# alxfox/AR_Voxel_Project

Hardware: AMD Instinct MI355X
Metric: Mvoxel-views/s (voxels x views / s) + carve wall-time, 512^3 grid x 36 views (higher is better)
Workload: dtype u8; 1 GPU; synthetic sphere silhouettes, 512x512x512 grid, 36 views 640x480, per step: derive bit planes + summed-area tables from the resident u8 masks, then dense carve of a fresh model by all views; one step after the other; views=36, jobs_in_flight=1, parallelism=single GPU, collective=none, cull=True

## Files before the change

ar_voxel_project_amd/capi.py:

```python
from __future__ import annotations

import ctypes as C
import os
from typing import Optional, Sequence, Tuple

import numpy as np

_HERE = os.path.dirname(os.path.abspath(__file__))
LIB_PATH = os.environ.get("ARVX_LIB_PATH") or os.path.join(_HERE, "lib", "libarvx.so")

OCC = 1
SEEN = 2
CARVE_NO_CULL = 1
CARVE_STATS = 2
CARVE_FUSED = 8
CARVE_STREAM = 16
CARVE_FILTER = 64
CARVE_NO_STREAM = 32
CARVE_DENSE_CLASSIFY = 128
CARVE_WHOLE_ITEMS = 256
PATH_DENSE_CLASSIFY = 1
PATH_ITEM_SHARING = 2
PATH_FRESH = 4
PATH_LAZY_CODES = 8
# ... 15 lines not shown
SYMBOLS = [
    "arvx_version", "arvx_last_error", "arvx_device_count", "arvx_projection_assoc",
    "arvx_ctx_create_slab_halo",
    "arvx_set_projection_assoc", "arvx_ctx_set_projection_assoc", "arvx_ctx_projection_assoc",
    "arvx_selftest_project", "arvx_selftest_depth", "arvx_selftest_view_tables",
    "arvx_ctx_create", "arvx_ctx_create_slab", "arvx_ctx_create_striped", "arvx_ctx_destroy",
    "arvx_ctx_set_stream", "arvx_ctx_set_exchange_stream", "arvx_ctx_synchronize", "arvx_ctx_voxels",
    "arvx_compose_projection", "arvx_set_views", "arvx_set_views_device",
    "arvx_set_images", "arvx_state_reset", "arvx_state_upload",
    "arvx_state_download", "arvx_state_device_ptr", "arvx_state_upload_halo",
    "arvx_state_upload_planes", "arvx_state_download_planes", "arvx_state_packet_geometry",
    "arvx_state_download_packets", "arvx_host_register",
    "arvx_host_unregister", "arvx_handle_unseen", "arvx_undistort", "arvx_undistort_device",
    "arvx_pack_occupancy", "arvx_pack_occupancy_global", "arvx_carve", "arvx_carve_views", "arvx_fast_carve",
    "arvx_color", "arvx_surface_count", "arvx_surface_download",
    "arvx_surface_depth_download", "arvx_color_samples",
    "arvx_color_visible", "arvx_surface_visible_download", "arvx_view_depth_download",
    "arvx_photo_carve", "arvx_carve_votes", "arvx_votes_download",
    "arvx_components", "arvx_components_download", "arvx_components_labels_download",
    "arvx_components_keep",
    "arvx_colors_upload", "arvx_closure", "arvx_closure_count", "arvx_closure_download",
    "arvx_closure_download32",
    "arvx_mc_cells", "arvx_mc_cells_download", "arvx_mc_mesh", "arvx_mc_mesh_download",
    "arvx_mc_mesh_download_faces", "arvx_mc_mesh_welded", "arvx_mc_mesh_welded_download",
    "arvx_mc_mesh_smooth", "arvx_mc_mesh_smooth_download",
    "arvx_mc_mesh_decimate", "arvx_mc_mesh_decimate_download",
    "arvx_render", "arvx_render_view", "arvx_render_download", "arvx_render_agreement",
    "arvx_occupancy_packet_words", "arvx_occupancy_compress", "arvx_occupancy_expand",
    "arvx_occupancy_expand_striped", "arvx_occupancy_pack_compress", "arvx_occupancy_expand_striped_others",
    "arvx_export_model", "arvx_get_stats", "arvx_last_carve_path", "arvx_last_fast_carve_path",
    "arvx_selftest_divide",
    "arvx_selftest_round",
    "arvx_ctx_set_rect_cache_limit", "arvx_selftest_rect_cache",
]


class ArvxError(RuntimeError):
    def __init__(self, code: int, msg: str):
        super().__init__(f"arvx error {code}: {msg}")
        self.code = code


class Stats(C.Structure):
    _fields_ = [
        ("subtiles", C.c_uint64),
        ("subtiles_carved", C.c_uint64),
        ("subtile_views_mixed", C.c_uint64),
        ("subtile_views_total", C.c_uint64),
        ("surface_voxels", C.c_uint64),
        ("reserved", C.c_uint64 * 3),
        ("host_total_fallbacks", C.c_uint64),
    ]


_libs: dict = {}
ASSOC_RIGHT, ASSOC_LEFT = 0, 1


def load_library(path: Optional[str] = None) -> C.CDLL:
    path = path or LIB_PATH
    if path in _libs:
        return _libs[path]
    if not os.path.exists(path):
        raise FileNotFoundError(
            f"{path} is missing: run `python -c 'import __graft_entry__ as g; g.build()'` "
            "(or make -C ar_voxel_project_amd/csrc); there is no CPU fallback")
# ... 38 lines not shown
        lib.arvx_state_download_packets.argtypes = [p, C.c_void_p, C.c_int64, C.c_void_p, C.c_int64,
                                                    C.POINTER(C.c_int64), C.POINTER(C.c_int64)]
        lib.arvx_host_register.argtypes = [C.c_void_p, C.c_size_t]
        lib.arvx_host_unregister.argtypes = [C.c_void_p]
        lib.arvx_handle_unseen.argtypes = [p]
    lib.arvx_state_upload_halo.argtypes = [p, u8p, u8p]
    lib.arvx_pack_occupancy.argtypes = [p, p]
    lib.arvx_pack_occupancy_global.argtypes = [p, p]
    lib.arvx_carve.argtypes = [p, C.c_uint]
    lib.arvx_carve_views.argtypes = [p, C.c_int, C.c_int, C.c_uint]
    lib.arvx_fast_carve.argtypes = [p]
    lib.arvx_color.argtypes = [p, C.c_int]
    lib.arvx_surface_count.argtypes = [p, C.POINTER(C.c_int64)]
    lib.arvx_surface_download.argtypes = [p, C.POINTER(C.c_int64), f32p]
    lib.arvx_surface_depth_download.argtypes = [p, f32p]
    lib.arvx_colors_upload.argtypes = [p, C.c_int64, C.POINTER(C.c_int64), f32p]
    lib.arvx_closure.argtypes = [p, C.c_int, C.c_int]
    lib.arvx_closure_count.argtypes = [p, C.POINTER(C.c_int64)]
    lib.arvx_closure_download.argtypes = [p, C.POINTER(C.c_int64), f32p]
    lib.arvx_export_model.argtypes = [p, f32p, C.c_int]
    lib.arvx_get_stats.argtypes = [p, C.POINTER(Stats)]
    if hasattr(lib, "arvx_last_carve_path"):
        lib.arvx_last_carve_path.argtypes = [p, C.POINTER(C.c_uint32)]
    if hasattr(lib, "arvx_last_fast_carve_path"):
        lib.arvx_last_fast_carve_path.argtypes = [p, C.POINTER(C.c_uint32)]
    ab_build = bool(os.environ.get("ARVX_LIB_PATH"))
    if hasattr(lib, "arvx_selftest_divide") or not ab_build:
        lib.arvx_selftest_divide.argtypes = [p, C.c_int64, f32p, f32p, f32p, f32p]
    if hasattr(lib, "arvx_selftest_round") or not ab_build:
        lib.arvx_selftest_round.argtypes = [p, C.POINTER(C.c_int64)]
    if hasattr(lib, "arvx_selftest_rect_cache") or not ab_build:
        lib.arvx_ctx_set_rect_cache_limit.argtypes = [p, C.c_uint64]
        lib.arvx_selftest_rect_cache.argtypes = [p, C.POINTER(C.c_int64)]
    if hasattr(lib, "arvx_mc_cells") or not ab_build:
        lib.arvx_mc_cells.argtypes = [p, C.POINTER(C.c_int64)]
        lib.arvx_mc_cells_download.argtypes = [p, C.POINTER(C.c_int32)]
    if hasattr(lib, "arvx_occupancy_compress") or not ab_build:
        lib.arvx_occupancy_packet_words.argtypes = [C.c_int64, C.c_int64]
        lib.arvx_occupancy_compress.argtypes = [p, C.c_void_p, C.c_int64, C.c_void_p, C.c_int64]
        lib.arvx_occupancy_expand.argtypes = [p, C.c_void_p, C.c_int, C.c_int, C.c_int64,
                                              C.c_int64, C.c_void_p, C.c_void_p]
        if hasattr(lib, "arvx_occupancy_expand_striped") or not ab_build:
            lib.arvx_occupancy_expand_striped.argtypes = [p, C.c_void_p, C.c_int, C.c_int64,
                                                          C.c_int64, C.c_int64, C.c_void_p,
                                                          C.c_void_p]
        if hasattr(lib, "arvx_occupancy_pack_compress"):
            lib.arvx_occupancy_pack_compress.argtypes = [p, C.c_void_p, C.c_int64, C.c_void_p]
            lib.arvx_occupancy_expand_striped_others.argtypes = [p, C.c_void_p, C.c_int, C.c_int, C.c_int64,
                                                                 C.c_int64, C.c_int64, C.c_void_p, C.c_void_p]
    if hasattr(lib, "arvx_mc_mesh_smooth"):
        lib.arvx_mc_mesh_smooth.argtypes = [p, C.c_int, C.c_float, C.c_float]
        lib.arvx_mc_mesh_smooth_download.argtypes = [p, C.c_void_p, C.c_void_p]
    if hasattr(lib, "arvx_mc_mesh_decimate"):
        lib.arvx_mc_mesh_decimate.argtypes = [p, C.c_int, C.c_int, C.POINTER(C.c_int64), C.POINTER(C.c_int64)]
        lib.arvx_mc_mesh_decimate_download.argtypes = [p, C.c_void_p, C.c_void_p, C.c_void_p, C.c_void_p,
                                                       C.c_void_p]
    if hasattr(lib, "arvx_color_visible"):
        lib.arvx_color_visible.argtypes = [p, C.c_int, C.c_float]
        lib.arvx_surface_visible_download.argtypes = [p, C.POINTER(C.c_int32)]
        lib.arvx_view_depth_download.argtypes = [p, C.c_int, f32p]
    if hasattr(lib, "arvx_photo_carve"):
        lib.arvx_photo_carve.argtypes = [p, C.c_float, C.c_int, C.c_float, C.c_int, C.POINTER(C.c_int),
                                         C.POINTER(C.c_int64)]
    if hasattr(lib, "arvx_carve_votes"):
        lib.arvx_carve_votes.argtypes = [p, C.c_int, C.c_uint]
        lib.arvx_votes_download.argtypes = [p, C.c_void_p, C.c_void_p]
# ... 16 lines not shown
            fn.restype = C.c_int64
        elif name not in ("arvx_last_error",):
            fn.restype = C.c_int
    _libs[path] = lib
    return lib


def occupancy_packet_words(n_words64: int, cap_words64: int) -> int:
    return int(load_library().arvx_occupancy_packet_words(n_words64, cap_words64))


def _check(rc: int, lib: Optional[C.CDLL] = None) -> None:
    if rc != 0:
        lib = lib or load_library()
        raise ArvxError(rc, lib.arvx_last_error().decode("utf-8", "replace"))


def _f32(a) -> np.ndarray:
    return np.ascontiguousarray(a, dtype=np.float32)


def _fp(a: np.ndarray):
    return a.ctypes.data_as(C.POINTER(C.c_float))


def compose_projection(K, Rt) -> np.ndarray:
    K = _f32(K).reshape(9)
    Rt = _f32(Rt).reshape(12)
    M = np.empty(12, np.float32)
    _check(load_library().arvx_compose_projection(_fp(K), _fp(Rt), _fp(M)))
    return M.reshape(3, 4)


def stripe_planes(Z: int, world: int, rank: int) -> np.ndarray:
    groups = np.arange(rank, Z // 8, world)
    return (groups[:, None] * 8 + np.arange(8)[None, :]).reshape(-1)


class Context:

    def __init__(self, X: int, Y: int, Z: int, voxel_size: float, device: int = 0,
                 z_range: Optional[Sequence[int]] = None,
                 stripes: Optional[Sequence[int]] = None, lib_path: Optional[str] = None,
                 assoc: Optional[int] = None, halo: int = 1):
        self._lib = load_library(lib_path)
        self._h = C.c_void_p()
        self.X, self.Y, self.Z = int(X), int(Y), int(Z)
        self.voxel_size = float(np.float32(voxel_size))
        if stripes is not None:
            world, rank = int(stripes[0]), int(stripes[1])
            self._ck(self._lib.arvx_ctx_create_striped(C.byref(self._h), device, X, Y, Z,
                                                     C.c_float(voxel_size), world, rank))
            self.planes = stripe_planes(Z, world, rank)
            self.z_range = None
        else:
            z0, z1 = (0, Z) if z_range is None else (int(z_range[0]), int(z_range[1]))
            self.z_range = (z0, z1)
            self._lib.arvx_ctx_create_slab_halo.argtypes = [
                C.POINTER(C.c_void_p), C.c_int, C.c_int, C.c_int, C.c_int, C.c_float, C.c_int,
                C.c_int, C.c_int]
            self._ck(self._lib.arvx_ctx_create_slab_halo(C.byref(self._h), device, X, Y, Z,
                                                       C.c_float(voxel_size), z0, z1, int(halo)))
            self.planes = np.arange(z0, z1)
        nz = len(self.planes)
        self.shape = (nz, Y, X)
        self.nvox = nz * Y * X
# ... 502 lines not shown
        return b, d, i

    def render_agreement(self, view: int) -> Tuple[int, int, int]:
        counts = (C.c_int64 * 3)()
        self._ck(self._lib.arvx_render_agreement(self._h, int(view), counts))
        self._render_wh = (self.W, self.H)
        return int(counts[0]), int(counts[1]), int(counts[2])

    def mc_mesh_count(self, apply_unseen: bool = False) -> int:
        n = C.c_int64()
        self._lib.arvx_mc_mesh.argtypes = [C.c_void_p, C.c_int, C.POINTER(C.c_int64)]
        self._ck(self._lib.arvx_mc_mesh(self._h, int(apply_unseen), C.byref(n)))
        return int(n.value)

    def export_model(self, apply_unseen: bool = False) -> np.ndarray:
        out = np.empty((self.nvox, 4), np.float32)
        self._ck(self._lib.arvx_export_model(self._h, _fp(out), int(apply_unseen)))
        return out

    def selftest_divide(self, a0, a1, b) -> np.ndarray:
        a0, a1, b = _f32(a0).reshape(-1), _f32(a1).reshape(-1), _f32(b).reshape(-1)
        out = np.empty((len(b), 4), np.float32)
        self._ck(self._lib.arvx_selftest_divide(self._h, len(b), _fp(a0), _fp(a1), _fp(b), _fp(out)))
        return out

    def selftest_round(self) -> int:
        n = C.c_int64(-1)
        self._ck(self._lib.arvx_selftest_round(self._h, C.byref(n)))
        return int(n.value)

    def set_rect_cache_limit(self, nbytes: int) -> None:
        self._ck(self._lib.arvx_ctx_set_rect_cache_limit(self._h, nbytes))

    def selftest_rect_cache(self) -> int:
        n = C.c_int64(-2)
        self._ck(self._lib.arvx_selftest_rect_cache(self._h, C.byref(n)))
        return int(n.value)

    def stats(self) -> dict:
        s = Stats()
        self._ck(self._lib.arvx_get_stats(self._h, C.byref(s)))
        out = {k: int(getattr(s, k)) for k, _ in Stats._fields_ if k != "reserved"}
        out["slices_evaluated"] = int(s.reserved[0])
        out["open_voxels_in_slices"] = int(s.reserved[1])
        out["mixed_pairs_uniform"] = int(s.reserved[2])
        out["host_total_fallbacks"] = int(s.host_total_fallbacks)
        return out
```

ar_voxel_project_amd/csrc/arvx_capi.hip:

```cpp
#include "arvx/arvx.h"

#include <hip/hip_runtime.h>

#include <cmath>
#include <cstdarg>
#include <cstdio>
#include <cstdlib>
#include <atomic>
#include <cstring>
#include <mutex>
#include <new>
#include <string>
#include <type_traits>
#include <utility>
#include <vector>

#include "arvx_ctx.h"
#include "carve_kernels.h"
#include "rect_cache_kernels.h"
#ifdef ARVX_EXPERIMENTS
#include "carve_stream_kernels.h"
#endif
#include "views_kernels.h"
#include "state_kernels.h"
// ... 486 lines not shown
    ARVX_SYNC(ctx);
    ctx->stream = hip_stream ? (hipStream_t)hip_stream : ctx->own_stream;
    ctx->carve_layout = 0;
    return ARVX_OK;
}

int arvx_ctx_set_exchange_stream(arvx_ctx *ctx, void *hip_stream) {
    ARVX_CHECK_CTX(ctx);
    ctx->xstream = (hipStream_t)hip_stream;
    return ARVX_OK;
}

#ifdef ARVX_EXPERIMENTS
extern "C" int arvx_experiment_mark_fault(arvx_ctx *ctx, unsigned mark) {
    if (!ctx || !ctx->h_fault) return fail(ARVX_ERR_INVALID, "null context");
    *ctx->h_fault = mark;
    return ARVX_OK;
}
#endif

int arvx_ctx_synchronize(arvx_ctx *ctx) {
    ARVX_CHECK_CTX(ctx);
    ARVX_HIP(hipStreamSynchronize(ctx->stream));
    return check_fault(ctx);
}

int arvx_ctx_voxels(const arvx_ctx *ctx, int64_t *count) {
    if (!ctx || !count) return fail(ARVX_ERR_INVALID, "null argument");
    *count = (int64_t)ctx->nvox;
    return ARVX_OK;
}


static int views_common(Ctx *ctx, int V, const float *M, const float *campos, int W, int H,
                        int C) {
    if (V < 1 || V > 4096) return fail(ARVX_ERR_INVALID, "V=%d out of range [1,4096]", V);
    if (!M) return fail(ARVX_ERR_INVALID, "null M");
    if (W < 1 || H < 1 || W > arvx::kMaxImageDim || H > arvx::kMaxImageDim)
        return fail(ARVX_ERR_INVALID, "image size %dx%d out of range", W, H);
    if (C < 1 || C > 4) return fail(ARVX_ERR_INVALID, "channels=%d out of range [1,4]", C);
    const bool same = ctx->M() && ctx->V == V && ctx->W == W && ctx->H == H;
    ctx->drop(Event::SetViews);
    ctx->views_ready = false;
    ctx->cameras_ready = false;
    if (!same) {
        ctx->free_views();
        ctx->pool_images.release();
    }
    ctx->images_ready = false;
    ctx->V = V;
    ctx->W = W;
    ctx->H = H;
    ctx->bgWords = (int)(((((size_t)W * H + 31) / 32 + 1) + 31) / 32 * 32);
    ctx->satW = (W + 1 + 63) / 64 * 64;
    ctx->satH = H + 1;
    ctx->satStride = ctx->satW * ctx->satH;
    if (!same) {
        hipError_t e = ctx->pool_M.reserve((size_t)V * 12 * sizeof(float));
        if (e == hipSuccess) e = ctx->pool_campos.reserve((size_t)V * 3 * sizeof(float));
        if (e == hipSuccess) e = ctx->pool_bg.reserve((size_t)V * ctx->bgWords * sizeof(uint32_t));
        if (e == hipSuccess) e = ctx->pool_sat.reserve((size_t)V * ctx->satStride * sizeof(uint16_t));
        if (e != hipSuccess) {
            ctx->free_views();
            return arvx::fail_hip(e, "hipMalloc(views)", __FILE__, __LINE__);
        }
    }
    const bool same_M = same && ctx->h_M.size() == (size_t)V * 12 &&
                        memcmp(ctx->h_M.data(), M, (size_t)V * 12 * sizeof(float)) == 0;
    if (!same_M) {
        ctx->rect_invalidate();
        ctx->h_M.assign(M, M + (size_t)V * 12);
        ARVX_HIP(hipMemcpyAsync(ctx->M(), ctx->h_M.data(), (size_t)V * 12 * sizeof(float),
                                hipMemcpyHostToDevice, ctx->stream));
    }
    ctx->has_campos = campos != nullptr;
    if (campos) {
        const bool same_c = same && ctx->h_campos.size() == (size_t)V * 3 &&
                            memcmp(ctx->h_campos.data(), campos, (size_t)V * 3 * sizeof(float)) == 0;
        if (!same_c) {
            ctx->h_campos.assign(campos, campos + (size_t)V * 3);
            ARVX_HIP(hipMemcpyAsync(ctx->campos(), ctx->h_campos.data(),
                                    (size_t)V * 3 * sizeof(float), hipMemcpyHostToDevice,
                                    ctx->stream));
        }
    } else {
        ctx->h_campos.clear();
    }
    return ARVX_OK;
}

static int views_preprocess(Ctx *ctx, const uint8_t *d_masks, int C) {
    const int npix = ctx->W * ctx->H;
    ARVX_HIP(hipGetLastError());
    static const bool three_launches = experiment_flag("ARVX_VIEWS_THREE_LAUNCHES");
    if ((C == 1 || C == 3) && ctx->W % 64 == 0 && ctx->W / 64 + 1 <= arvx::kStripMaxWaves && ctx->H <= 4096 &&
        ((uintptr_t)d_masks & 15u) == 0 && !three_launches) {
        const int TIs = (ctx->H + 63) / 64;
        const size_t G = (size_t)ctx->W / 2;
        const size_t off_gran = ((size_t)ctx->V * sizeof(unsigned long long) + 255) / 256 * 256;
        const size_t vbytes = off_gran + (size_t)ctx->V * TIs * G * sizeof(unsigned long long);
        const size_t key = ((size_t)ctx->V << 40) ^ ((size_t)TIs << 24) ^ G;
        if (ctx->vstrip_key != key || ctx->pool_vstrip.cap < vbytes) {
            ARVX_HIP(ctx->pool_vstrip.reserve(vbytes));
            ARVX_HIP(hipMemsetAsync(ctx->pool_vstrip.p, 0, vbytes, ctx->stream));
            ctx->vstrip_key = key;
        }
        unsigned long long *ctr = (unsigned long long *)ctx->pool_vstrip.p;
        unsigned long long *gran = (unsigned long long *)((uint8_t *)ctx->pool_vstrip.p + off_gran);
        if (C == 1)
            hipLaunchKernelGGL(arvx::views_strip_kernel<1>, dim3(TIs, ctx->V), dim3(64 * (ctx->W / 64 + 1)),
                               0, ctx->stream, d_masks, ctx->W, ctx->H, TIs, ctx->bg(), ctx->bgWords,
                               ctx->sat(), ctx->satStride, ctx->satW, ctr, gran, ctx->d_fault);
        else
            hipLaunchKernelGGL(arvx::views_strip_kernel<3>, dim3(TIs, ctx->V), dim3(64 * (ctx->W / 64 + 1)),
                               0, ctx->stream, d_masks, ctx->W, ctx->H, TIs, ctx->bg(), ctx->bgWords,
                               ctx->sat(), ctx->satStride, ctx->satW, ctr, gran, ctx->d_fault);
        ARVX_HIP(hipGetLastError());
        ctx->views_ready = true;
        ctx->cameras_ready = true;
        return ARVX_OK;
    }
    if (C == 1 && npix % 32 == 0 && ((uintptr_t)d_masks & 15u) == 0) {
        hipLaunchKernelGGL(arvx::views_bits16_kernel, dim3((npix / 16 + 255) / 256, ctx->V),
                           dim3(256), 0, ctx->stream, d_masks, npix, ctx->bg(), ctx->bgWords);
    } else if (C == 1 || C == 3) {
        const dim3 g1(((npix + 3) / 4 + 255) / 256, ctx->V);
        if (C == 1)
            hipLaunchKernelGGL(arvx::views_bits_kernel<1>, g1, dim3(256), 0, ctx->stream, d_masks,
                               npix, ctx->bg(), ctx->bgWords);
        else
            hipLaunchKernelGGL(arvx::views_bits_kernel<3>, g1, dim3(256), 0, ctx->stream, d_masks,
                               npix, ctx->bg(), ctx->bgWords);
    } else {
        const dim3 g1((npix + 255) / 256, ctx->V);
        hipLaunchKernelGGL(arvx::views_bits_generic_kernel, g1, dim3(256), 0, ctx->stream, d_masks,
                           C, npix, ctx->bg(), ctx->bgWords);
    }
    ARVX_HIP(hipGetLastError());
    const int W = ctx->W, H = ctx->H, V = ctx->V;
    const int TJ = (W + 1 + 63) / 64, TI = (H + arvx::kTileRows - 1) / arvx::kTileRows;
    const size_t n_rs = (size_t)V * H * TJ, n_T = (size_t)V * TI * TJ * 64, n_ts = (size_t)V * TI * TJ;
    ARVX_HIP(ctx->pool_scratch.reserve((n_rs + n_T + n_ts) * sizeof(int) + 64));
    int *d_rs = (int *)ctx->pool_scratch.p, *d_T = d_rs + n_rs, *d_ts = d_T + n_T;
    const unsigned tgrid = (unsigned)(((size_t)TJ * TI * V + 3) / 4);
    hipLaunchKernelGGL(arvx::views_tile_sums_kernel, dim3(tgrid), dim3(256), 0, ctx->stream,
                       ctx->bg(), ctx->bgWords, W, H, TJ, TI, V, d_rs, d_T, d_ts);
    hipLaunchKernelGGL(arvx::views_table_kernel, dim3(tgrid), dim3(256), 0, ctx->stream,
                       ctx->bg(), ctx->bgWords, W, H, TJ, TI, V, d_rs, d_T, d_ts, ctx->sat(),
                       ctx->satStride, ctx->satW);
    ARVX_HIP(hipGetLastError());
    ctx->views_ready = true;
    ctx->cameras_ready = true;
    return ARVX_OK;
}

int arvx_set_views(arvx_ctx *ctx, int V, const float *M, const float *campos,
                   const uint8_t *const *masks, int W, int H, int C, size_t stride) {
    ARVX_CHECK_CTX(ctx);
    if (!masks) {
        if (int rc0 = views_common(ctx, V, M, campos, W, H, C > 0 ? C : 1)) return rc0;
        ctx->cameras_ready = true;
        ARVX_SYNC(ctx);
        return ARVX_OK;
    }
    if (W >= 1 && C >= 1 && stride < (size_t)W * C)
        return fail(ARVX_ERR_INVALID, "stride %zu < W*C", stride);
    for (int i = 0; i < V; ++i)
        if (!masks[i]) return fail(ARVX_ERR_INVALID, "null mask %d", i);
    int rc = views_common(ctx, V, M, campos, W, H, C);
    if (rc) return rc;
    const size_t img = (size_t)W * H * C;
    ARVX_HIP(ctx->pool_raw_masks.reserve(img * V));
    uint8_t *d_raw = (uint8_t *)ctx->pool_raw_masks.p;
    bool packed = stride == (size_t)W * C;
    for (int i = 1; i < V && packed; ++i) packed = masks[i] == masks[i - 1] + img;
    if (packed) {
        ARVX_HIP(hipMemcpyAsync(d_raw, masks[0], img * V, hipMemcpyHostToDevice, ctx->stream));
    } else {
        for (int i = 0; i < V; ++i)
            ARVX_HIP(hipMemcpy2DAsync(d_raw + img * i, (size_t)W * C, masks[i], stride,
                                      (size_t)W * C, H, hipMemcpyHostToDevice, ctx->stream));
    }
    rc = views_preprocess(ctx, d_raw, C);
    if (rc) return rc;
    ARVX_SYNC(ctx);
// ... 1833 lines not shown
                          const int32_t *xyz, float *rows_uv) {
    ARVX_CHECK_CTX(ctx);
    if (!M) return fail(ARVX_ERR_INVALID, "null M");
    arvx::SelftestMatrix m;
    memcpy(m.m, M, sizeof m.m);
    const unsigned grid = (unsigned)((n + 255) / 256);
    return selftest_xyz(ctx, n, xyz, (size_t)n * 5, rows_uv, [&](int *d_xyz, float *d_out) {
        by_assoc(ctx, [&](auto left) {
            hipLaunchKernelGGL(arvx::selftest_project_kernel<decltype(left)::value>, dim3(grid), dim3(256), 0,
                               ctx->stream, m, voxel_size, d_xyz, (long long)n, d_out, d_out + 3 * n);
        });
    });
}

int arvx_selftest_depth(arvx_ctx *ctx, int64_t n, const float campos[3], float voxel_size,
                        const int32_t *xyz, float *depth) {
    ARVX_CHECK_CTX(ctx);
    if (!campos) return fail(ARVX_ERR_INVALID, "null campos");
    arvx::SelftestMatrix m;
    memset(&m, 0, sizeof m);
    memcpy(m.m, campos, 3 * sizeof(float));
    return selftest_xyz(ctx, n, xyz, (size_t)n, depth, [&](int *d_xyz, float *d_out) {
        hipLaunchKernelGGL(arvx::selftest_depth_kernel, dim3((unsigned)((n + 255) / 256)), dim3(256),
                           0, ctx->stream, m, voxel_size, d_xyz, (long long)n, d_out);
    });
}

int arvx_selftest_view_tables(arvx_ctx *ctx, int view, uint32_t *bg_bits, uint16_t *table, int *ld) {
    ARVX_CHECK_CTX(ctx);
    if (!ctx->views_ready) return fail(ARVX_ERR_STATE, "arvx_set_views has not been called");
    if (view < 0 || view >= ctx->V) return fail(ARVX_ERR_INVALID, "view %d outside [0,%d)", view, ctx->V);
    if (!ld) return fail(ARVX_ERR_INVALID, "null ld");
    *ld = ctx->satW;
    const size_t words = ((size_t)ctx->W * ctx->H + 31) / 32;
    if (bg_bits)
        ARVX_HIP(hipMemcpyAsync(bg_bits, ctx->bg() + (size_t)view * ctx->bgWords, words * sizeof(uint32_t),
                                hipMemcpyDeviceToHost, ctx->stream));
    if (table)
        ARVX_HIP(hipMemcpyAsync(table, ctx->sat() + (size_t)view * ctx->satStride,
                                (size_t)ctx->satStride * sizeof(uint16_t), hipMemcpyDeviceToHost,
                                ctx->stream));
    ARVX_SYNC(ctx);
    return ARVX_OK;
}

int arvx_selftest_round(arvx_ctx *ctx, int64_t *mismatches) {
    ARVX_CHECK_CTX(ctx);
    if (!mismatches) return fail(ARVX_ERR_INVALID, "null mismatches");
    *mismatches = -1;
    ARVX_HIP(ctx->pool_scratch.reserve(64));
    unsigned long long *d_bad = (unsigned long long *)ctx->pool_scratch.p;
    ARVX_HIP(hipMemsetAsync(d_bad, 0, sizeof *d_bad, ctx->stream));
    const unsigned ranges[2][2] = {{0x00000000u, 0x4B800000u}, {0x80000000u, 0xBEFFFFFFu}};
    for (const auto &r : ranges) {
        const unsigned long long n = (unsigned long long)r[1] - r[0] + 1;
        hipLaunchKernelGGL(arvx::selftest_round_kernel, dim3((unsigned)((n + 255) / 256)), dim3(256),
                           0, ctx->stream, r[0], r[1], d_bad);
        ARVX_HIP(hipGetLastError());
    }
    unsigned long long bad = 0;
    ARVX_HIP(hipMemcpyAsync(&bad, d_bad, sizeof bad, hipMemcpyDeviceToHost, ctx->stream));
    ARVX_SYNC(ctx);
    *mismatches = (int64_t)bad;
    return ARVX_OK;
}

int arvx_ctx_set_rect_cache_limit(arvx_ctx *ctx, uint64_t bytes) {
    ARVX_CHECK_CTX(ctx);
    if (bytes > (uint64_t)1 << 46) return fail(ARVX_ERR_INVALID, "limit of %llu bytes", (unsigned long long)bytes);
    if (ctx->pool_rect.p) ARVX_SYNC(ctx);
    ctx->pool_rect.release();
    ctx->rect_state = Ctx::Rect::None;
    ctx->rect_limit = (size_t)bytes;
    return ARVX_OK;
// ... 1028 lines not shown
```

ar_voxel_project_amd/csrc/arvx_ctx.h:

```cpp
#pragma once

#include <hip/hip_runtime.h>
#include <stdint.h>

#include <vector>

namespace arvx {

int fail_hip(hipError_t e, const char *what, const char *file, int line);
int fail_msg(int code, const char *msg);

#define ARVX_HIP(call)                                                        \
    do {                                                                      \
        hipError_t arvx_e_ = (call);                                          \
        if (arvx_e_ != hipSuccess)                                            \
            return ::arvx::fail_hip(arvx_e_, #call, __FILE__, __LINE__);      \
    } while (0)

struct DevPool {
    enum Size { Headroom, Exact };
    void *p = nullptr;
    size_t cap = 0;
    const bool exact;
    explicit DevPool(Size size = Headroom) : exact(size == Exact) {}
// ... 97 lines not shown
    int64_t timeline_n = 0;
    int timeline_rec = 32;
    DevPool pool_flood_rec{DevPool::Exact};
    DevPool pool_flood_code;
    DevPool pool_coarse{DevPool::Exact};
    DevPool pool_stats{DevPool::Exact};
    unsigned long long *stats() const { return (unsigned long long *)pool_stats.p; }
    unsigned long long host_total_fallbacks = 0;
    DevPool pool_scratch{DevPool::Exact};
    DevPool pool_xscratch;
    DevPool pool_flood{DevPool::Exact};

    bool views_ready = false;
    bool cameras_ready = false;
    bool has_campos = false;
    int V = 0, W = 0, H = 0;
    int bgWords = 0, satStride = 0;
    int satW = 0, satH = 0;
    DevPool pool_M{DevPool::Exact}, pool_campos{DevPool::Exact}, pool_bg{DevPool::Exact},
        pool_sat{DevPool::Exact};
    float *M() const { return (float *)pool_M.p; }
    float *campos() const { return (float *)pool_campos.p; }
    uint32_t *bg() const { return (uint32_t *)pool_bg.p; }
    uint16_t *sat() const { return (uint16_t *)pool_sat.p; }
    std::vector<float> h_M, h_campos;
    enum class Rect { None, Built, Refused };
    Rect rect_state = Rect::None;
    int rect_streak = 0;
    size_t rect_limit = (size_t)1 << 30;
    DevPool pool_rect{DevPool::Exact};
    void rect_invalidate() {
        rect_state = Rect::None;
        rect_streak = 0;
    }

    DevPool pool_images{DevPool::Exact};
    uint8_t *images() const { return (uint8_t *)pool_images.p; }
    bool images_ready = false;
    int *d_surf_index = nullptr;
    float4 *d_surf_rgba = nullptr;
    float *d_surf_depth = nullptr;
    uint8_t *d_surf_has = nullptr;
    int64_t surf_count = 0;
    std::vector<int> h_surf_index;
    std::vector<uint8_t> h_surf_has;
    bool color_ready = false;
    DevPool pool_col_bits, pool_col_rank;
    bool color_visible = false;
    long long vis_large_need = 0;
    DevPool pool_vis_depth{DevPool::Exact}, pool_vis_large{DevPool::Exact}, pool_vis_views;
    DevPool pool_photo_rm, pool_photo_plane{DevPool::Exact};
    DevPool pool_votes{DevPool::Exact};
    bool votes_ready = false;

    DevPool pool_comp_label{DevPool::Exact}, pool_comp_planes{DevPool::Exact}, pool_comp_rank{DevPool::Exact},
        pool_comp_table, pool_comp_ctl;
    bool comp_ready = false;
    int comp_conn = 0;
    long long comp_count = 0, comp_cap = 0;

    int *d_clo_index = nullptr;
    void *d_clo_rgba = nullptr;
    int64_t clo_count = 0;
    bool closure_ready = false;
    int closure_unseen = 0;
    bool closure_fills = false;
    int closure_radius = 0;
// ... 104 lines not shown
```

ar_voxel_project_amd/csrc/views_kernels.h:

```cpp
#pragma once

#include "arvx_device.h"

namespace arvx {

template <int C>
__global__ __launch_bounds__(256) void views_bits_kernel(const uint8_t *__restrict__ masks,
                                                         int npix, uint32_t *__restrict__ bg,
                                                         int bgWords) {
    const int v = blockIdx.y;
    const int q = blockIdx.x * 256 + threadIdx.x;
    uint32_t *dst = bg + (size_t)v * bgWords;
    if (q == 0) dst[bgWords - 1] = 0;
    const uint8_t *src = masks + ((size_t)v * npix + 4 * (size_t)q) * C;
    uint32_t nib = 0;
    if (4 * q + 3 < npix && (((uintptr_t)src) & 3u) == 0) {
        uint32_t w[C];
#pragma unroll
        for (int c = 0; c < C; ++c) w[c] = reinterpret_cast<const uint32_t *>(src)[c];
        const uint8_t *b = reinterpret_cast<const uint8_t *>(w);
#pragma unroll
        for (int j = 0; j < 4; ++j) {
            bool isbg = true;
#pragma unroll
// ... 185 lines not shown
        const uint32_t t = (((d[k] & 0x7f7f7f7fu) + 0x7f7f7f7fu) | d[k]) & 0x80808080u;
        f |= bytes_to_nibble(t >> 7) << (4 * k);
    }
    return f;
}
__device__ __forceinline__ uint32_t nonzero_bytes(const uint32_t x) {
    return ((((x & 0x7f7f7f7fu) + 0x7f7f7f7fu) | x) >> 7) & 0x01010101u;
}

__device__ __forceinline__ uint32_t nonzero16x3(const uint4 a, const uint4 b, const uint4 c) {
    const uint32_t d[12] = {a.x, a.y, a.z, a.w, b.x, b.y, b.z, b.w, c.x, c.y, c.z, c.w};
    uint32_t m[2] = {0u, 0u};
#pragma unroll
    for (int k = 0; k < 12; ++k) {
        const uint32_t t = (((d[k] & 0x7f7f7f7fu) + 0x7f7f7f7fu) | d[k]) & 0x80808080u;
        m[k / 6] |= bytes_to_nibble(t >> 7) << (4 * (k % 6));
    }
    uint32_t f = 0;
#pragma unroll
    for (int h = 0; h < 2; ++h) {
        uint32_t x = (m[h] | (m[h] >> 1) | (m[h] >> 2)) & 0x249249u;
        x = (x | (x >> 2)) & 0x0C30C3u;
        x = (x | (x >> 4)) & 0x00F00Fu;
        x = (x | (x >> 8)) & 0xFFu;
        f |= x << (8 * h);
    }
    return f;
}

template <int C>
__global__ __launch_bounds__(64 * kStripMaxWaves) void views_strip_kernel(
    const uint8_t *__restrict__ masks, int W, int H, int TI, uint32_t *__restrict__ bg, int bgWords,
    uint16_t *__restrict__ sat, int satStride, int ld, unsigned long long *__restrict__ ctr,
    unsigned long long *__restrict__ gran, unsigned *__restrict__ err) {
    __shared__ unsigned long long s_bits[64 * (kStripMaxWaves - 1)];
    __shared__ int s_rowcnt[kStripMaxWaves][64];
    __shared__ uint16_t s_col[kStripMaxWaves][64];
    __shared__ int s_tot[kStripMaxWaves];
    __shared__ uint4 s_row[kStripMaxWaves][64];
    __shared__ unsigned long long s_ticket;
    const int v = blockIdx.y;
    if (threadIdx.x == 0) s_ticket = atomicAdd(&ctr[v], 1ull);
    __syncthreads();
    const unsigned long long ticket = s_ticket;
    const int I = (int)(ticket % (unsigned long long)TI);
    const uint32_t tag = (uint32_t)(ticket / (unsigned long long)TI) + 1u;
    const int J = threadIdx.x >> 6, lane = threadIdx.x & 63;
    const int TP = W >> 6;
    const int G = W >> 1;
    const uint8_t *img = masks + (size_t)v * W * H * C;
    const int y0 = I * 64;
    const int nrows = min(64, H - y0);
    const int rr = lane >> 2, q = lane & 3;

    uint32_t mine_lo = 0, mine_hi = 0;
    uint32_t acc[4] = {0u, 0u, 0u, 0u};
    if (J < TP) {
        uint4 w[4][C];
#pragma unroll
        for (int k = 0; k < 4; ++k) {
            const int y = y0 + 4 * rr + k;
            const uint4 *src = reinterpret_cast<const uint4 *>(img + ((size_t)y * W + 64 * J + 16 * q) * C);
#pragma unroll
            for (int c = 0; c < C; ++c) w[k][c] = (y < H) ? src[c] : make_uint4(0u, 0u, 0u, 0u);
        }
#pragma unroll
        for (int k = 0; k < 4; ++k) {
// ... 64 lines not shown
    }

    int above = 0;
    if (J < TP && I > 0) {
        const unsigned long long *g0 = gran + (size_t)v * TI * G + 32 * J + (lane >> 1);
        for (unsigned spin = 0;; ++spin) {
            bool ok = true;
            int sum = 0;
            for (int k = 0; k < I; ++k) {
                const unsigned long long g = granule_load(g0 + (size_t)k * G);
                ok = ok && (uint32_t)(g >> 32) == tag;
                sum += (int)(((uint32_t)g >> (16 * (lane & 1))) & 0xffffu);
            }
            if (__all(ok)) {
                above = sum;
                break;
            }
            if (spin > (1u << 20)) {
                if (lane == 0) __hip_atomic_store(err, 1u, __ATOMIC_RELAXED, __HIP_MEMORY_SCOPE_SYSTEM);
                break;
            }
            __builtin_amdgcn_s_sleep(8);
        }
    }
    int sc = above;
#pragma unroll
    for (int d = 1; d < 64; d <<= 1) {
        const int t = __shfl_up(sc, d);
        if (lane >= d) sc += t;
    }
    if (lane == 63) s_tot[J] = sc;
    __syncthreads();

    int left = 0, lt = 0;
    for (int k = 0; k < J; ++k) {
        left += s_rowcnt[k][lane];
        lt += s_tot[k];
    }
    uint16_t *tab = sat + (size_t)v * satStride;
    const unsigned off = 64u * (unsigned)J + (unsigned)lane;
    if (I == 0) tab[off] = 0;
    uint4 *const rows = s_row[J];
    rows[lane] = make_uint4(mine_lo, mine_hi, (uint32_t)left, 0u);
    wave_lds_fence();
    uint32_t run = (uint32_t)(sc - above + lt);
    uint16_t *row = tab + (size_t)(y0 + 1) * ld;
#pragma unroll 4
    for (int r = 0; r < nrows; ++r) {
        const uint4 f = rows[r];
        run = __builtin_amdgcn_mbcnt_hi(f.y, __builtin_amdgcn_mbcnt_lo(f.x, run)) + f.z;
        row[off] = (uint16_t)run;
        row += ld;
    }
}

}
```

include/arvx/arvx.h:

```cpp
#ifndef ARVX_H
#define ARVX_H

#include <stddef.h>
#include <stdint.h>

#ifdef __cplusplus
extern "C" {
#endif

#define ARVX_VERSION 100

enum {
    ARVX_OK = 0,
    ARVX_ERR_INVALID = 1,
    ARVX_ERR_HIP = 2,
    ARVX_ERR_STATE = 3,
    ARVX_ERR_NOMEM = 4
};

#define ARVX_OCC 1u
#define ARVX_SEEN 2u

#define ARVX_CARVE_NO_CULL 1u
#define ARVX_CARVE_STATS 2u
// ... 160 lines not shown

int arvx_get_stats(arvx_ctx *ctx, arvx_stats *out);

#define ARVX_PATH_DENSE_CLASSIFY 1u
#define ARVX_PATH_ITEM_SHARING 2u
#define ARVX_PATH_FRESH 4u
#define ARVX_PATH_LAZY_CODES 8u
#define ARVX_PATH_FUSED 16u
#define ARVX_PATH_BRUTE_FORCE 32u
#define ARVX_PATH_STREAM 64u
#define ARVX_PATH_RECT_BLOCKS 128u
int arvx_last_carve_path(arvx_ctx *ctx, uint32_t out[4]);

#define ARVX_FLOOD_PREPASS 1u
#define ARVX_FLOOD_FRESH 2u
int arvx_last_fast_carve_path(arvx_ctx *ctx, uint32_t out[4]);

int arvx_selftest_divide(arvx_ctx *ctx, int64_t n, const float *a0, const float *a1,
                         const float *b, float *out);

int arvx_selftest_project(arvx_ctx *ctx, int64_t n, const float M[12], float voxel_size,
                          const int32_t *xyz, float *rows_uv);
int arvx_selftest_depth(arvx_ctx *ctx, int64_t n, const float campos[3], float voxel_size,
                        const int32_t *xyz, float *depth);

int arvx_selftest_view_tables(arvx_ctx *ctx, int view, uint32_t *bg_bits, uint16_t *table, int *ld);

int arvx_selftest_round(arvx_ctx *ctx, int64_t *mismatches);

int arvx_ctx_set_rect_cache_limit(arvx_ctx *ctx, uint64_t bytes);

int arvx_selftest_rect_cache(arvx_ctx *ctx, int64_t *mismatches);

#ifdef __cplusplus
}
#endif
#endif
```

Baseline: 52.77 million Mvoxel-views/s.

## Skip summed-area table writes outside each view's projected grid window

Computes a conservative per-view image window from the projection of the grid bounding box, with error margins, on the host. The window is cached and uploaded as packed tile ranges. The strip kernel then returns early for tiles outside that window, skipping their summed-area table row writes. Tables are marked partial and fully rebuilt from the bit planes when a caller downloads them. This trades host-side bound computation and extra bookkeeping for fewer table stores, and it relies on the carve never reading table entries outside the window.

```diff
diff --git a/ar_voxel_project_amd/capi.py b/ar_voxel_project_amd/capi.py
--- a/ar_voxel_project_amd/capi.py
+++ b/ar_voxel_project_amd/capi.py
@@ -71,6 +71,8 @@
     "arvx_selftest_divide",
     "arvx_selftest_round",
     "arvx_ctx_set_rect_cache_limit", "arvx_selftest_rect_cache",
+    "arvx_ctx_set_view_window", "arvx_view_window", "arvx_view_window_host",
+    "arvx_selftest_fill_view_tables", "arvx_selftest_view_table_raw",
 ]
 
 
@@ -175,6 +177,13 @@
     if hasattr(lib, "arvx_selftest_rect_cache") or not ab_build:
         lib.arvx_ctx_set_rect_cache_limit.argtypes = [p, C.c_uint64]
         lib.arvx_selftest_rect_cache.argtypes = [p, C.POINTER(C.c_int64)]
+    if hasattr(lib, "arvx_view_window") or not ab_build:
+        lib.arvx_ctx_set_view_window.argtypes = [p, C.c_int]
+        lib.arvx_view_window.argtypes = [p, C.c_int, C.POINTER(C.c_int)]
+        lib.arvx_view_window_host.argtypes = [C.c_int, C.c_int, C.c_int, C.c_float, f32p, C.c_int, C.c_int,
+                                              C.POINTER(C.c_int)]
+        lib.arvx_selftest_fill_view_tables.argtypes = [p, C.c_int]
+        lib.arvx_selftest_view_table_raw.argtypes = [p, C.c_int, C.c_void_p]
     if hasattr(lib, "arvx_mc_cells") or not ab_build:
         lib.arvx_mc_cells.argtypes = [p, C.POINTER(C.c_int64)]
         lib.arvx_mc_cells_download.argtypes = [p, C.POINTER(C.c_int32)]
@@ -257,6 +266,13 @@
     return M.reshape(3, 4)
 
 
+def view_window_host(X: int, Y: int, Z: int, voxel_size: float, M, W: int, H: int) -> Tuple[int, int, int, int]:
+    M = _f32(M).reshape(12)
+    rect = (C.c_int * 4)()
+    _check(load_library().arvx_view_window_host(X, Y, Z, C.c_float(voxel_size), _fp(M), W, H, rect))
+    return tuple(int(r) for r in rect)
+
+
 def stripe_planes(Z: int, world: int, rank: int) -> np.ndarray:
     groups = np.arange(rank, Z // 8, world)
     return (groups[:, None] * 8 + np.arange(8)[None, :]).reshape(-1)
@@ -825,6 +841,26 @@
     def set_rect_cache_limit(self, nbytes: int) -> None:
         self._ck(self._lib.arvx_ctx_set_rect_cache_limit(self._h, nbytes))
 
+    def set_view_window(self, on: bool) -> None:
+        self._ck(self._lib.arvx_ctx_set_view_window(self._h, int(bool(on))))
+
+    def view_window(self, view: int) -> Tuple[int, int, int, int]:
+        rect = (C.c_int * 4)()
+        self._ck(self._lib.arvx_view_window(self._h, view, rect))
+        return tuple(int(r) for r in rect)
+
+    def selftest_fill_view_tables(self, value: int) -> None:
+        self._ck(self._lib.arvx_selftest_fill_view_tables(self._h, int(value)))
+
+    def selftest_view_table_raw(self, view: int, H: int) -> np.ndarray:
+        ld = C.c_int()
+        self._lib.arvx_selftest_view_tables.argtypes = [C.c_void_p, C.c_int, C.c_void_p, C.c_void_p,
+                                                        C.POINTER(C.c_int)]
+        self._ck(self._lib.arvx_selftest_view_tables(self._h, view, None, None, C.byref(ld)))
+        table = np.zeros((H + 1, ld.value), np.uint16)
+        self._ck(self._lib.arvx_selftest_view_table_raw(self._h, view, table.ctypes.data))
+        return table
+
     def selftest_rect_cache(self) -> int:
         n = C.c_int64(-2)
         self._ck(self._lib.arvx_selftest_rect_cache(self._h, C.byref(n)))
diff --git a/ar_voxel_project_amd/csrc/arvx_capi.hip b/ar_voxel_project_amd/csrc/arvx_capi.hip
--- a/ar_voxel_project_amd/csrc/arvx_capi.hip
+++ b/ar_voxel_project_amd/csrc/arvx_capi.hip
@@ -542,6 +542,122 @@
 }
 
 
+static bool view_window(int X, int Y, int Z, float s, const float *M, int W, int H, int win[4]) {
+    const int TI = (H + 63) / 64, JL = W / 64;
+    win[0] = 0;
+    win[1] = TI - 1;
+    win[2] = 0;
+    win[3] = JL;
+    const double wy[2] = {0.0, (double)((float)(Y - 1) * s)};
+    const double wx[2] = {0.0, (double)((float)(X - 1) * s)};
+    const double wz[2] = {0.0, (double)((float)(-(Z - 1)) * s)};
+    double E[3], lo[3], hi[3];
+    double a[3][8];
+    for (int r = 0; r < 3; ++r) {
+        const double m0 = M[4 * r], m1 = M[4 * r + 1], m2 = M[4 * r + 2], m3 = M[4 * r + 3];
+        E[r] = std::fabs(m0) * std::fabs(wy[1]) + std::fabs(m1) * std::fabs(wx[1]) +
+               std::fabs(m2) * std::fabs(wz[1]) + std::fabs(m3);
+        for (int c = 0; c < 8; ++c) a[r][c] = m0 * wy[c & 1] + m1 * wx[(c >> 1) & 1] + m2 * wz[c >> 2] + m3;
+    }
+    double cmin = INFINITY, cmax = -INFINITY;
+    for (int c = 0; c < 8; ++c) {
+        cmin = std::fmin(cmin, a[2][c]);
+        cmax = std::fmax(cmax, a[2][c]);
+    }
+    const double k19 = 1.001 / 524288.0, k20 = 1.0 / 1048576.0, k12 = 1.0 / 4096.0;
+    const double eps0 = E[0] * k19, eps1 = E[1] * k19, eps2 = E[2] * k19;
+    if (!(cmin > 0.0 || cmax < 0.0)) return true;
+    const double cabs = cmin > 0.0 ? cmin : -cmax;
+    if (!(cabs > 16.0 * eps2 + 1e-30)) return true;
+    const double D = cabs - 2.0 * eps2;
+    for (int r = 0; r < 2; ++r) {
+        lo[r] = INFINITY;
+        hi[r] = -INFINITY;
+        for (int c = 0; c < 8; ++c) {
+            const double u = a[r][c] / a[2][c];
+            lo[r] = std::fmin(lo[r], u);
+            hi[r] = std::fmax(hi[r], u);
+        }
+    }
+    int t0[2], t1[2];
+    for (int r = 0; r < 2; ++r) {
+        const double Ua = std::fmax(std::fabs(lo[r]), std::fabs(hi[r]));
+        if (!(Ua < 1.0e6)) return true;
+        const double epsr = r == 0 ? eps0 : eps1;
+        const double err = (epsr + Ua * eps2) / D + Ua * k20 + k12;
+        const double Ub = Ua + err;
+        const double mu = 1.001 * (epsr + Ub * eps2) / D + Ub * k20 + k12;
+        const double n = r == 0 ? (double)W : (double)H;
+        double l = std::floor(lo[r] - err - mu - 0.5) - 1.0;
+        double h = std::ceil(hi[r] + err + mu + 0.5) + 1.0 + 1.0;
+        if (!(l == l && h == h)) return true;
+        l = std::fmin(std::fmax(l, 0.0), n);
+        h = std::fmin(std::fmax(h, l), n);
+        t0[r] = (int)l;
+        t1[r] = (int)h;
+    }
+    win[2] = t0[0] / 64;
+    win[3] = t1[0] / 64;
+    win[0] = t0[1] <= 1 ? 0 : (t0[1] - 1) / 64;
+    win[1] = t1[1] <= 1 ? 0 : (t1[1] - 1) / 64;
+    return win[0] == 0 && win[1] == TI - 1 && win[2] == 0 && win[3] == JL;
+}
+static uint32_t window_word(const int win[4]) {
+    return (uint32_t)win[0] | ((uint32_t)win[1] << 8) | ((uint32_t)win[2] << 16) | ((uint32_t)win[3] << 24);
+}
+static void window_rect(uint32_t w, int H, int satW, int rect[4]) {
+    const int I0 = (int)(w & 0xffu), I1 = (int)((w >> 8) & 0xffu), J0 = (int)((w >> 16) & 0xffu), J1 = (int)(w >> 24);
+    rect[0] = I0 == 0 ? 0 : 64 * I0 + 1;
+    rect[1] = std::min(H, 64 * (I1 + 1));
+    rect[2] = 64 * J0;
+    rect[3] = std::min(satW - 1, 64 * J1 + 63);
+}
+
+int arvx_view_window_host(int X, int Y, int Z, float voxel_size, const float M[12], int W, int H,
+                          int rect[4]) {
+    if (!M || !rect) return fail(ARVX_ERR_INVALID, "null argument");
+    if (X < 1 || Y < 1 || Z < 1 || !(voxel_size > 0.f)) return fail(ARVX_ERR_INVALID, "bad grid");
+    if (W < 1 || H < 1 || W > arvx::kMaxImageDim || H > arvx::kMaxImageDim)
+        return fail(ARVX_ERR_INVALID, "image size %dx%d out of range", W, H);
+    int win[4];
+    view_window(X, Y, Z, voxel_size, M, W, H, win);
+    window_rect(window_word(win), H, (W + 1 + 63) / 64 * 64, rect);
+    return ARVX_OK;
+}
+
+static int views_windows(Ctx *ctx, bool strip) {
+    const int V = ctx->V;
+    if (!ctx->win_valid) {
+        ctx->h_win_geo.resize(V);
+        for (int v = 0; v < V; ++v) {
+            int win[4];
+            view_window(ctx->X, ctx->Y, ctx->Z, ctx->s, ctx->h_M.data() + 12 * (size_t)v, ctx->W, ctx->H, win);
+            ctx->h_win_geo[v] = window_word(win);
+        }
+        ctx->win_valid = true;
+    }
+    const int whole[4] = {0, (ctx->H + 63) / 64 - 1, 0, ctx->W / 64};
+    const uint32_t all = window_word(whole);
+    const bool geo = strip && ctx->win_on;
+    bool same = ctx->h_win.size() == (size_t)V && ctx->pool_win.cap >= (size_t)V * sizeof(uint32_t);
+    ctx->sat_partial = false;
+    for (int v = 0; v < V; ++v) {
+        const uint32_t w = geo ? ctx->h_win_geo[v] : all;
+        if (w != all) ctx->sat_partial = true;
+        same = same && ctx->h_win[v] == w;
+    }
+    if (!same) {
+        ARVX_HIP(ctx->pool_win.reserve((size_t)V * sizeof(uint32_t)));
+        if (geo)
+            ctx->h_win = ctx->h_win_geo;
+        else
+            ctx->h_win.assign(V, all);
+        ARVX_HIP(hipMemcpyAsync(ctx->pool_win.p, ctx->h_win.data(), (size_t)V * sizeof(uint32_t),
+                                hipMemcpyHostToDevice, ctx->stream));
+    }
+    return ARVX_OK;
+}
+
 static int views_common(Ctx *ctx, int V, const float *M, const float *campos, int W, int H,
                         int C) {
     if (V < 1 || V > 4096) return fail(ARVX_ERR_INVALID, "V=%d out of range [1,4096]", V);
@@ -599,6 +715,7 @@
     return ARVX_OK;
 }
 
+static int views_tables_from_bits(Ctx *ctx);
 static int views_preprocess(Ctx *ctx, const uint8_t *d_masks, int C) {
     const int npix = ctx->W * ctx->H;
     ARVX_HIP(hipGetLastError());
@@ -617,19 +734,22 @@
         }
         unsigned long long *ctr = (unsigned long long *)ctx->pool_vstrip.p;
         unsigned long long *gran = (unsigned long long *)((uint8_t *)ctx->pool_vstrip.p + off_gran);
+        if (int rc = views_windows(ctx, true)) return rc;
+        const uint32_t *win = (const uint32_t *)ctx->pool_win.p;
         if (C == 1)
             hipLaunchKernelGGL(arvx::views_strip_kernel<1>, dim3(TIs, ctx->V), dim3(64 * (ctx->W / 64 + 1)),
                                0, ctx->stream, d_masks, ctx->W, ctx->H, TIs, ctx->bg(), ctx->bgWords,
-                               ctx->sat(), ctx->satStride, ctx->satW, ctr, gran, ctx->d_fault);
+                               ctx->sat(), ctx->satStride, ctx->satW, ctr, gran, ctx->d_fault, win);
         else
             hipLaunchKernelGGL(arvx::views_strip_kernel<3>, dim3(TIs, ctx->V), dim3(64 * (ctx->W / 64 + 1)),
                                0, ctx->stream, d_masks, ctx->W, ctx->H, TIs, ctx->bg(), ctx->bgWords,
-                               ctx->sat(), ctx->satStride, ctx->satW, ctr, gran, ctx->d_fault);
+                               ctx->sat(), ctx->satStride, ctx->satW, ctr, gran, ctx->d_fault, win);
         ARVX_HIP(hipGetLastError());
         ctx->views_ready = true;
         ctx->cameras_ready = true;
         return ARVX_OK;
     }
+    if (int rc = views_windows(ctx, false)) return rc;
     if (C == 1 && npix % 32 == 0 && ((uintptr_t)d_masks & 15u) == 0) {
         hipLaunchKernelGGL(arvx::views_bits16_kernel, dim3((npix / 16 + 255) / 256, ctx->V),
                            dim3(256), 0, ctx->stream, d_masks, npix, ctx->bg(), ctx->bgWords);
@@ -647,6 +767,13 @@
                            C, npix, ctx->bg(), ctx->bgWords);
     }
     ARVX_HIP(hipGetLastError());
+    if (int rc = views_tables_from_bits(ctx)) return rc;
+    ctx->views_ready = true;
+    ctx->cameras_ready = true;
+    return ARVX_OK;
+}
+
+static int views_tables_from_bits(Ctx *ctx) {
     const int W = ctx->W, H = ctx->H, V = ctx->V;
     const int TJ = (W + 1 + 63) / 64, TI = (H + arvx::kTileRows - 1) / arvx::kTileRows;
     const size_t n_rs = (size_t)V * H * TJ, n_T = (size_t)V * TI * TJ * 64, n_ts = (size_t)V * TI * TJ;
@@ -659,8 +786,38 @@
                        ctx->bg(), ctx->bgWords, W, H, TJ, TI, V, d_rs, d_T, d_ts, ctx->sat(),
                        ctx->satStride, ctx->satW);
     ARVX_HIP(hipGetLastError());
-    ctx->views_ready = true;
-    ctx->cameras_ready = true;
+    return ARVX_OK;
+}
+
+static int complete_tables(Ctx *ctx) {
+    if (!ctx->sat_partial) return ARVX_OK;
+    if (int rc = views_tables_from_bits(ctx)) return rc;
+    ctx->sat_partial = false;
+    return ARVX_OK;
+}
+
+int arvx_ctx_set_view_window(arvx_ctx *ctx, int on) {
+    ARVX_CHECK_CTX(ctx);
+    ctx->win_on = on != 0;
+    return ARVX_OK;
+}
+
+int arvx_view_window(arvx_ctx *ctx, int view, int rect[4]) {
+    ARVX_CHECK_CTX(ctx);
+    if (!rect) return fail(ARVX_ERR_INVALID, "null rect");
+    if (!ctx->views_ready || ctx->h_win.size() != (size_t)ctx->V)
+        return fail(ARVX_ERR_STATE, "arvx_set_views has not been called");
+    if (view < 0 || view >= ctx->V) return fail(ARVX_ERR_INVALID, "view %d outside [0,%d)", view, ctx->V);
+    window_rect(ctx->h_win[view], ctx->H, ctx->satW, rect);
+    return ARVX_OK;
+}
+
+int arvx_selftest_fill_view_tables(arvx_ctx *ctx, int value) {
+    ARVX_CHECK_CTX(ctx);
+    if (!ctx->views_ready) return fail(ARVX_ERR_STATE, "arvx_set_views has not been called");
+    ARVX_HIP(hipMemsetAsync(ctx->sat(), value & 0xff, (size_t)ctx->V * ctx->satStride * sizeof(uint16_t),
+                            ctx->stream));
+    ctx->views_ready = false;
     return ARVX_OK;
 }
 
@@ -2560,6 +2717,8 @@
     if (view < 0 || view >= ctx->V) return fail(ARVX_ERR_INVALID, "view %d outside [0,%d)", view, ctx->V);
     if (!ld) return fail(ARVX_ERR_INVALID, "null ld");
     *ld = ctx->satW;
+    if (table)
+        if (int rc = complete_tables(ctx)) return rc;
     const size_t words = ((size_t)ctx->W * ctx->H + 31) / 32;
     if (bg_bits)
         ARVX_HIP(hipMemcpyAsync(bg_bits, ctx->bg() + (size_t)view * ctx->bgWords, words * sizeof(uint32_t),
@@ -2568,6 +2727,17 @@
         ARVX_HIP(hipMemcpyAsync(table, ctx->sat() + (size_t)view * ctx->satStride,
                                 (size_t)ctx->satStride * sizeof(uint16_t), hipMemcpyDeviceToHost,
                                 ctx->stream));
+    ARVX_SYNC(ctx);
+    return ARVX_OK;
+}
+
+int arvx_selftest_view_table_raw(arvx_ctx *ctx, int view, uint16_t *table) {
+    ARVX_CHECK_CTX(ctx);
+    if (!ctx->views_ready) return fail(ARVX_ERR_STATE, "arvx_set_views has not been called");
+    if (view < 0 || view >= ctx->V) return fail(ARVX_ERR_INVALID, "view %d outside [0,%d)", view, ctx->V);
+    if (!table) return fail(ARVX_ERR_INVALID, "null table");
+    ARVX_HIP(hipMemcpyAsync(table, ctx->sat() + (size_t)view * ctx->satStride,
+                            (size_t)ctx->satStride * sizeof(uint16_t), hipMemcpyDeviceToHost, ctx->stream));
     ARVX_SYNC(ctx);
     return ARVX_OK;
 }
diff --git a/ar_voxel_project_amd/csrc/arvx_ctx.h b/ar_voxel_project_amd/csrc/arvx_ctx.h
--- a/ar_voxel_project_amd/csrc/arvx_ctx.h
+++ b/ar_voxel_project_amd/csrc/arvx_ctx.h
@@ -153,7 +153,14 @@
     void rect_invalidate() {
         rect_state = Rect::None;
         rect_streak = 0;
-    }
+        win_valid = false;
+    }
+    bool win_on = true;
+    bool win_valid = false;
+    bool sat_partial = false;
+    std::vector<uint32_t> h_win_geo;
+    std::vector<uint32_t> h_win;
+    DevPool pool_win{DevPool::Exact};
 
     DevPool pool_images{DevPool::Exact};
     uint8_t *images() const { return (uint8_t *)pool_images.p; }
diff --git a/ar_voxel_project_amd/csrc/views_kernels.h b/ar_voxel_project_amd/csrc/views_kernels.h
--- a/ar_voxel_project_amd/csrc/views_kernels.h
+++ b/ar_voxel_project_amd/csrc/views_kernels.h
@@ -241,7 +241,8 @@
 __global__ __launch_bounds__(64 * kStripMaxWaves) void views_strip_kernel(
     const uint8_t *__restrict__ masks, int W, int H, int TI, uint32_t *__restrict__ bg, int bgWords,
     uint16_t *__restrict__ sat, int satStride, int ld, unsigned long long *__restrict__ ctr,
-    unsigned long long *__restrict__ gran, unsigned *__restrict__ err) {
+    unsigned long long *__restrict__ gran, unsigned *__restrict__ err,
+    const uint32_t *__restrict__ win) {
     __shared__ unsigned long long s_bits[64 * (kStripMaxWaves - 1)];
     __shared__ int s_rowcnt[kStripMaxWaves][64];
     __shared__ uint16_t s_col[kStripMaxWaves][64];
@@ -372,6 +373,13 @@
     if (lane == 63) s_tot[J] = sc;
     __syncthreads();
 
+    {
+        const uint32_t w = win[v];
+        const int Ju = __builtin_amdgcn_readfirstlane(J);
+        const bool inside = I >= (int)(w & 0xffu) && I <= (int)((w >> 8) & 0xffu) &&
+                            Ju >= (int)((w >> 16) & 0xffu) && Ju <= (int)(w >> 24);
+        if (!inside) return;
+    }
     int left = 0, lt = 0;
     for (int k = 0; k < J; ++k) {
         left += s_rowcnt[k][lane];
diff --git a/include/arvx/arvx.h b/include/arvx/arvx.h
--- a/include/arvx/arvx.h
+++ b/include/arvx/arvx.h
@@ -216,6 +216,14 @@
 
 int arvx_selftest_rect_cache(arvx_ctx *ctx, int64_t *mismatches);
 
+int arvx_ctx_set_view_window(arvx_ctx *ctx, int on);
+int arvx_view_window(arvx_ctx *ctx, int view, int rect[4]);
+int arvx_view_window_host(int X, int Y, int Z, float voxel_size, const float M[12], int W, int H,
+                          int rect[4]);
+
+int arvx_selftest_fill_view_tables(arvx_ctx *ctx, int value);
+int arvx_selftest_view_table_raw(arvx_ctx *ctx, int view, uint16_t *table);
+
 #ifdef __cplusplus
 }
 #endif
```

Measured after the change: 53.92 million Mvoxel-views/s, median of 6. 2.2% higher.
